# jglaser/metadynamics-plugin

Hardware: AMD Instinct MI355X
Metric: particle_cv_evals_per_s (higher is better)
Workload: dtype f32; 1 GPU; 1xMI355X: 10^6 particles, 2 lamellar CVs (8 Fourier modes each), 256^2 bias grid, well-tempered; particles_per_gpu=1000000, particles_global=1000000, n_cv=2, modes_per_cv=8, grid=256x256, stride=1, fast_trig=1, fast_trig_library_default=1, driver=host, mode=single

## Files before the change

### metadynamics-plugin_amd/csrc/fused.hip

```cpp
#include <hip/hip_runtime.h>
#include <hip/hip_ext.h>

#ifdef MTD_STAMPS
__device__ unsigned long long g_stamps[64];
#define MTD_STAMP(slot, cond)                                                   \
    do                                                                          \
        {                                                                       \
        if (cond) g_stamps[slot] = wall_clock64();                              \
        } while (0)
extern "C" int mtd_debug_read_stamps(unsigned long long *host)
    {
    return (int)hipMemcpyFromSymbol(host, HIP_SYMBOL(g_stamps), sizeof(unsigned long long) * 64);
    }
#else
#define MTD_STAMP(slot, cond) do { } while (0)
#endif

#include "lamellar_host.hpp"
#include "metad_host.hpp"
#include "comm_host.hpp"

#include <cstdlib>
#include <cstring>
#include <map>
#include <mutex>
#include <utility>
#include <vector>

namespace
{

using namespace mtd;

constexpr int FCV_THREADS = 512;
constexpr int FCV_UNROLL = 4;
constexpr int FF_THREADS = 256;
constexpr int FF_UNROLL = 2;

template<typename S4, int NCV, bool FAST, bool COMM, bool ORTHO, int U = FCV_UNROLL>
__global__ __launch_bounds__(FCV_THREADS) void k_fused_cv(const LamKArgs a, const S4 *__restrict__ postype, const unsigned int N,
                                                          double *partials, const MetadCfg c,
                                                          const unsigned int n_apply_blocks, const CommK ck)
    {
    __shared__ float s_coeff[MTD_MAX_CV * MTD_MAX_TYPES];
    __shared__ double s_wave[(FCV_THREADS / MTD_WAVE) * NCV];
    __shared__ double s_red[16];
    __shared__ ModeTables s_mt;

    MTD_STAMP(0, blockIdx.x == 0 && threadIdx.x == 0);
    MTD_STAMP(3, blockIdx.x == n_apply_blocks && threadIdx.x == 0);
    if (blockIdx.x < n_apply_blocks)
        {
        const unsigned int b0 = blockIdx.x * FCV_THREADS;
        apply_cells(c, b0, min(c.len, b0 + FCV_THREADS), blockIdx.x == 0, s_red);
// ... 49 lines not shown
template<> struct ff_groups<float4, 1, false> { static constexpr int value = 2; };
template<> struct ff_groups<double4, 1, true> { static constexpr int value = 2; };
template<> struct ff_groups<double4, 1, false> { static constexpr int value = 2; };

template<typename S4, int NCV, bool FAST, int GROUPS, bool COMM, bool ORTHO>
__global__ __launch_bounds__(FF_THREADS, 4) void k_fused_force(const FusedEntry e, const LamKArgs a, const ForcePtrs out,
                                                            const double two_over_n, const MetadCfg c, const int deposit, const CommK ck)
    {
    __shared__ ChainResult s_chain;
    __shared__ float s_wcoef[MTD_MAX_CV * MTD_MAX_TYPES];
    __shared__ double s_red[16];
    __shared__ ModeTables s_mt;

    const int wave = threadIdx.x >> 6;
    const int lane = threadIdx.x & 63;
    const unsigned int n_grid_blocks = fused_entry_read(e);
    const unsigned int n_blocks = e.n_particle_blocks;
    const S4 *__restrict__ postype = (const S4 *)e.postype;
    const unsigned int N = e.N;
    const unsigned int n_modes = e.n_modes;
    const bool grid_block = blockIdx.x < n_grid_blocks;
    const unsigned int block_id = blockIdx.x - n_grid_blocks;
    const unsigned int stride = n_blocks * FF_STREAM_THREADS;
    const unsigned int first = block_id * FF_STREAM_THREADS + (wave - 1) * MTD_WAVE + lane;
    const unsigned int first1 = first + FF_U * stride;

    ForceRegs<NCV, FF_U> R, R1;
    MTD_STAMP(16, blockIdx.x == 0 && threadIdx.x == 0);
    MTD_STAMP(24, blockIdx.x == n_grid_blocks && threadIdx.x == 0);
    constexpr int NCH = CHAIN_MAX_CV;
    ChainPre<NCH> pre;
    int pre_meta = 0;
    constexpr bool early = !COMM;
    float4 th = make_float4(0.f, 0.f, 0.f, 0.f), tq = th;
    float tc = 0.0f;
    if (wave == 0)
        {
        if (!grid_block)
            {
            static_assert(MTD_MAX_MODES >= MTD_WAVE && MTD_MAX_CV * MTD_MAX_TYPES >= MTD_WAVE, "a lane is a valid index");
            th = a.h[lane];
            tq = a.q[lane];
            tc = (&a.coeff[0][0])[lane];
            }
        if (early)
            pre_meta = chain_preload<NCH>(e, pre);
        else
            pre_meta = chain_preload<NCH, false>(e, pre);
        }
    RawGroup<S4, FF_U> raw0;
    if (wave != 0 && !grid_block && N) lam_force_request<S4, FF_U>(postype, N, first, stride, raw0);
    if (!grid_block)
        {
        if (wave == 0)
            {
            if (lane < (int)n_modes)
                {
                s_mt.h[lane] = th;
                s_mt.q[lane] = tq;
                }
            if (lane < NCV * MTD_MAX_TYPES) s_wcoef[lane] = tc;
            }
        lds_barrier();
        }
    MTD_STAMP(25, blockIdx.x == n_grid_blocks && threadIdx.x == 0);
    if (wave == 0)
        {
        ChainResult r;
        chain_preload_resolve<NCH>(pre_meta, pre);
        if constexpr (early)
            {
            double vi[3];
#pragma unroll
            for (int i = 0; i < NCH; ++i) vi[i] = (pre.x[i][0] + pre.x[i][1]) + (pre.x[i][2] + pre.x[i][3]);
            r = chain_wave(c, deposit != 0, true, nullptr, nullptr, false, &pre.patch, pre.patch_ok != 0, true, vi[0], vi[1], vi[2]);
            }
        else
            r = chain_wave(c, deposit != 0, true, &ck, nullptr, false, &pre.patch, pre.patch_ok != 0);
        MTD_STAMP(17, blockIdx.x == 0 && threadIdx.x == 0);
        MTD_STAMP(26, blockIdx.x == n_grid_blocks && threadIdx.x == 0);
        if (lane == 0) chain_share(s_chain, r);
        if (!grid_block && lane < NCV * MTD_MAX_TYPES)
            {
            const unsigned int cv = lane / MTD_MAX_TYPES;
            const unsigned int gs = cv < a.n_cv ? a.slot[cv] : 0u;
            const double b = gs == 0 ? r.bias[0] : (gs == 1 ? r.bias[1] : r.bias[2]);
            s_wcoef[lane] = (cv < a.n_cv) ? (float)((double)s_wcoef[lane] * b * two_over_n) : 0.0f;
            }
        }
    else if (!grid_block && N)
        {
        RawGroup<S4, FF_U> raw1;
        if (GROUPS > 1) lam_force_request<S4, FF_U>(postype, N, first1, stride, raw1);
        lam_force_unscaled_from<S4, NCV, FAST, FF_U, ORTHO>(a, N, first, stride, s_mt, raw0, R);
        if (GROUPS > 1) lam_force_unscaled_from<S4, NCV, FAST, FF_U, ORTHO>(a, N, first1, stride, s_mt, raw1, R1);
        MTD_STAMP(27, blockIdx.x == n_grid_blocks && threadIdx.x == 64);
        }
    lds_barrier();
    MTD_STAMP(18, blockIdx.x == 0 && threadIdx.x == 0);
    MTD_STAMP(28, blockIdx.x == n_grid_blocks && threadIdx.x == 64);

    if (grid_block)
        {
        const double2 sums = grid_first_pass_cells_256(c, s_chain, blockIdx.x);
        MTD_STAMP(19, blockIdx.x == 0 && threadIdx.x == 0);
        grid_first_pass_sums_256(c, blockIdx.x, sums, s_red);
        MTD_STAMP(20, blockIdx.x == 0 && threadIdx.x == 0);
        }
// ... 101 lines not shown
std::mutex g_force_profile_mutex;

bool force_profile_next(hipEvent_t &start, hipEvent_t &stop)
    {
    std::lock_guard<std::mutex> lock(g_force_profile_mutex);
    ForceProfile &p = g_force_profile;
    if (p.used + 2 > p.ev.size()) return false;
    start = p.ev[p.used];
    stop = p.ev[p.used + 1];
    p.used += 2;
    return true;
    }

template<typename F> int with_fused_cv_kernel(int dtype, bool fast, bool ortho, bool comm, unsigned int n_cv, F &&f)
    {
    return dispatch_s4_fast(dtype, fast, [&](auto s4, auto fast_c)
        {
        using S4 = typename decltype(s4)::type;
        constexpr bool FAST = decltype(fast_c)::value;
        return dispatch_bool(ortho, [&](auto ortho_c)
            {
            constexpr bool ORTHO = decltype(ortho_c)::value;
            if (comm)
                return dispatch_count<CHAIN_MAX_CV>(n_cv, [&](auto n) { return f(k_fused_cv<S4, decltype(n)::value, FAST, true, ORTHO>, s4); });
            return dispatch_count<MAXCV>(n_cv, [&](auto n) { return f(k_fused_cv<S4, decltype(n)::value, FAST, false, ORTHO>, s4); });
            });
        });
    }

}

namespace mtd
{
unsigned int resident_capacity(const void *kernel, int threads)
    {
    static std::mutex mu;
    static std::map<std::pair<int, const void *>, unsigned int> cache;
    int per_cu = 0, dev = 0, n_cu = 0;
    if (hipGetDevice(&dev) != hipSuccess)
        {
        (void)hipGetLastError();
        return 0;
        }
    std::lock_guard<std::mutex> lock(mu);
    auto it = cache.find(std::make_pair(dev, kernel));
    if (it != cache.end()) return it->second;
    unsigned int cap = 0;
    if (hipDeviceGetAttribute(&n_cu, hipDeviceAttributeMultiprocessorCount, dev) == hipSuccess &&
        hipOccupancyMaxActiveBlocksPerMultiprocessor(&per_cu, kernel, threads, 0) == hipSuccess)
        cap = (unsigned int)per_cu * (unsigned int)n_cu;
    else
        (void)hipGetLastError();
    cache[std::make_pair(dev, kernel)] = cap;
    return cap;
    }
}

extern "C" {

int mtd_fused_cv_pass(mtd_metad *m, const mtd_lamellar_set *set, unsigned int n_particles, const void *d_postype,
                      int dtype, const mtd_box *global_box, double *d_partials, unsigned int *n_partials,
                      mtd_stream_t stream)
    {
    if (!m) return MTD_ERR_INVALID_ARGUMENT;
    if (m->h_step_err && *m->h_step_err) return MTD_ERR_COMM_TIMEOUT;
    LamKArgs k;
    int rc = fill_kargs(k, set, global_box);
    if (rc) return rc;
    if (!d_partials || !n_partials || (n_particles && !d_postype)) return MTD_ERR_INVALID_ARGUMENT;
    if (dtype != MTD_F32 && dtype != MTD_F64) return MTD_ERR_INVALID_ARGUMENT;
    if (set->n_cv > (unsigned int)MAXCV) return MTD_ERR_UNSUPPORTED;
    hipStream_t s = (hipStream_t)stream;
    const unsigned int blocks = lam_cv_blocks(n_particles);
    *n_partials = blocks;
    const unsigned int n_apply = m->pending_apply ? (m->cfg.len + FCV_THREADS - 1) / FCV_THREADS : 0;
    const bool fast = lam_fast_trig(k) != 0;
    if (m->comm && (set->n_cv > (unsigned int)CHAIN_MAX_CV || set->n_cv != m->cfg.n_cv)) return MTD_ERR_UNSUPPORTED;
    const LamKArgs kd = dense_cv_args(k);
    rc = with_fused_cv_kernel(dtype, fast, k.ortho != 0, m->comm != nullptr, set->n_cv, [&](auto kernel, auto s4) -> int
        {
        using S4 = typename decltype(s4)::type;
        const unsigned int grid = blocks + n_apply;
        CommK ck;
        std::memset(&ck, 0, sizeof(ck));
        if (m->comm)
            {
            if (grid > resident_capacity((const void *)kernel, FCV_THREADS)) return MTD_ERR_UNSUPPORTED;
            const int rcn = comm_next(m->comm, ck);
            if (rcn) return rcn;
            }
        kernel<<<grid, FCV_THREADS, 0, s>>>(kd, (const S4 *)d_postype, n_particles, d_partials, m->cfg, n_apply, ck);
// ... 190 lines not shown
```

### metadynamics-plugin_amd/csrc/metad.hip

```cpp
#include "metad_device.hpp"

#include <cmath>
#include <cstring>
#include <mutex>
#include <new>

#include "metad_host.hpp"
#include "comm_host.hpp"

#include <cstdlib>

namespace
{

using namespace mtd;

__global__ __launch_bounds__(GRID_THREADS) void k_prepare(const MetadCfg c, const int deposit)
    {
    __shared__ EvalShared sh;
    __shared__ double s_tmp[16];
    reduce_cv_sources(c, sh.cv, s_tmp);
    __syncthreads();
    evaluate_bias(c, sh, deposit != 0, false);
    if (threadIdx.x < c.n_cv) c.st->cv[threadIdx.x] = sh.cv[threadIdx.x];
// ... 516 lines not shown
int mtd_metad_update_phase_a(mtd_metad *m, unsigned int timestep, int *deposited, mtd_stream_t stream)
    {
    if (!m || !deposited) return MTD_ERR_INVALID_ARGUMENT;
    { int frc = mtd::metad_flush(m, (hipStream_t)stream); if (frc) return frc; }
    hipStream_t s = (hipStream_t)stream;
    const int dep = deposit_due(m, timestep);
    k_prepare<<<1, GRID_THREADS, 0, s>>>(m->cfg, dep);
    MTD_LAUNCH_CHECK();
    if (dep)
        {
        k_reweight1<true, false><<<m->cfg.n_gblocks, GRID_THREADS, 0, s>>>(m->cfg);
        MTD_LAUNCH_CHECK();
        }
    *deposited = dep;
    return MTD_SUCCESS;
    }

int mtd_metad_update_phase_b(mtd_metad *m, int deposited, mtd_stream_t stream)
    {
    if (!m) return MTD_ERR_INVALID_ARGUMENT;
    hipStream_t s = (hipStream_t)stream;
    if (deposited)
        {
        k_reweight1<false, true><<<m->cfg.n_gblocks, GRID_THREADS, 0, s>>>(m->cfg);
        MTD_LAUNCH_CHECK();
        k_apply<<<m->cfg.n_gblocks, GRID_THREADS, 0, s>>>(m->cfg);
        MTD_LAUNCH_CHECK();
        }
    k_evaluate<<<1, GRID_THREADS, 0, s>>>(m->cfg);
    MTD_LAUNCH_CHECK();
    return MTD_SUCCESS;
    }

void mtd_debug_walker_check_pack(unsigned int stride, int add_bias, unsigned int timestep, double *out12)
    {
    const unsigned int q[3] = { stride, (unsigned int)(add_bias != 0), timestep };
    for (int i = 0; i < 3; ++i)
        {
        const double lo = (double)(q[i] & 0xffffu), hi = (double)(q[i] >> 16);
        out12[4 * i] = lo;
        out12[4 * i + 1] = lo * lo;
        out12[4 * i + 2] = hi;
        out12[4 * i + 3] = hi * hi;
        }
    }

int mtd_debug_walker_check_verify(const double *sums12, const double *mine12, unsigned int world)
    {
    const double W = (double)world;
    for (int i = 0; i < 12; ++i)
        if (sums12[i] != W * mine12[i]) return 0;
    return 1;
    }

int mtd_metad_update_bias_walkers(mtd_metad *m, mtd_rccl *walkers, unsigned int timestep, mtd_stream_t stream)
    {
    if (!m) return MTD_ERR_INVALID_ARGUMENT;
    int rc;
    if (walkers && (m->walkers_checked != (const void *)walkers || m->walkers_stride != m->stride || m->walkers_add_bias != m->add_bias))
        {
        double *d_chk = nullptr;
        MTD_HIP_TRY(hipMalloc(&d_chk, 12 * sizeof(double)));
        double mine[12], h[12];
        mtd_debug_walker_check_pack(m->stride, m->add_bias, timestep, mine);
        hipError_t e = hipMemcpyAsync(d_chk, mine, sizeof(mine), hipMemcpyHostToDevice, (hipStream_t)stream);
        rc = e == hipSuccess ? mtd_comm_allreduce_large(walkers, d_chk, 12, MTD_ELEM_F64, stream) : (int)e;
// ... 164 lines not shown
```

### metadynamics-plugin_amd/csrc/metad_device.hpp

```cpp
#pragma once

#include "mtd_device.hpp"
#include "comm_device.hpp"
#include "exact_div.hpp"

#include <cstddef>

#ifndef MTD_STAMP
#define MTD_STAMP(slot, cond) do { } while (0)
#endif

namespace mtd
{

constexpr int MAXCV = MTD_METAD_MAX_CV;
constexpr int GRID_THREADS = 256;
constexpr int MAX_POINTS = 2 * MAXCV + 2;
constexpr int MAX_TERMS = 1 << MAXCV;

struct CvSource
    {
    const double *partials;
    unsigned int n_partials, stride, offset, _pad;
    double scale, shift;
// ... 382 lines not shown
                    {
                    const int coord = gp.org[i] + rest % 6;
                    rest /= 6;
                    in = in && coord >= 0 && coord < (int)c.lengths[i];
                    cell += (unsigned int)coord * c.factors[i];
                    }
            if (in) gp.v[r] = c.grid[cell];
            }
        }
    return gp;
    }

template<int NCH> struct ChainPre
    {
    double x[NCH][4];
    GridPatch patch;
    int patch_ok;
    };

struct ChainSums
    {
    const double *ptr[CHAIN_MAX_CV];
    unsigned int cnt[CHAIN_MAX_CV], str[CHAIN_MAX_CV], off[CHAIN_MAX_CV];
    };

struct alignas(64) FusedEntry
    {
    const void *postype;
    MetadState *st;
    unsigned int N;
    unsigned int n_particle_blocks;
    unsigned int n_passenger_blocks;
    unsigned int n_modes, n_cv;
    unsigned int _pad;
    ChainSums sums;
    };
static_assert(sizeof(FusedEntry) <= 128 && alignof(FusedEntry) == 64, "one aligned batch of scalar loads");
static_assert(CHAIN_MAX_CV == 3 && sizeof(ChainSums) == 64 && offsetof(FusedEntry, sums) == 40, "fused_entry_read names every field");

__device__ __forceinline__ unsigned int fused_entry_read_head(const FusedEntry &e)
    {
    unsigned int npb;
    asm("s_mov_b32 %0, %1" : "=s"(npb) : "s"(e.n_passenger_blocks), "s"(e.postype), "s"(e.st), "s"(e.N), "s"(e.n_particle_blocks),
        "s"(e.n_modes), "s"(e.n_cv));
    return npb;
    }
__device__ __forceinline__ unsigned int fused_entry_read(const FusedEntry &e)
    {
    unsigned int npb;
    asm("s_mov_b32 %0, %1" : "=s"(npb) : "s"(e.n_passenger_blocks), "s"(e.postype), "s"(e.st), "s"(e.N), "s"(e.n_particle_blocks),
        "s"(e.n_modes), "s"(e.n_cv), "s"(e.sums.ptr[0]), "s"(e.sums.ptr[1]), "s"(e.sums.ptr[2]), "s"(e.sums.cnt[0]), "s"(e.sums.cnt[1]),
        "s"(e.sums.cnt[2]), "s"(e.sums.str[0]), "s"(e.sums.str[1]), "s"(e.sums.str[2]), "s"(e.sums.off[0]), "s"(e.sums.off[1]),
        "s"(e.sums.off[2]));
    return npb;
    }

inline ChainSums chain_sums_of(const MetadCfg &c)
    {
    ChainSums s;
    const double *safe = &c.st->zero;
#pragma unroll
    for (int i = 0; i < CHAIN_MAX_CV; ++i)
        {
        const bool on = i < (int)c.n_cv && c.src[i].partials != nullptr;
        s.ptr[i] = on ? c.src[i].partials : safe;
        s.cnt[i] = on ? c.src[i].n_partials : 0u;
        s.str[i] = on ? c.src[i].stride : 0u;
        s.off[i] = on ? c.src[i].offset : 0u;
        }
    return s;
    }

template<int NCH, bool SUMS>
__device__ __forceinline__ void chain_preload_sums(const ChainSums &s, const double *safe, ChainPre<NCH> &p)
    {
    const unsigned int lane = threadIdx.x & 63;
#pragma unroll
    for (int i = 0; i < NCH; ++i)
#pragma unroll
        for (int j = 0; j < 4; ++j)
            {
            const unsigned int b = lane + j * MTD_WAVE;
            const double *q = (SUMS && b < s.cnt[i]) ? s.ptr[i] + ((size_t)b * s.str[i] + s.off[i]) : safe;
            p.x[i][j] = SUMS ? *q : 0.0;
// ... 33 lines not shown
#pragma unroll
        for (int j = 0; j < 4; ++j)
            {
            const unsigned int b = lane + j * MTD_WAVE;
            const double *q = (SUMS && b < cnt[i]) ? ptr[i] + ((size_t)b * str[i] + off[i]) : safe;
            p.x[i][j] = SUMS ? *q : 0.0;
            }
    p.patch_ok = ok;
#pragma unroll
    for (int i = 0; i < CHAIN_MAX_CV; ++i) p.patch.org[i] = org[i];
    p.patch.v[0] = c.st->patch_v[lane];
#pragma unroll
    for (int r = 1; r < 4; ++r) p.patch.v[r] = NCH == 3 ? c.st->patch_v[min(lane + 64 * r, 215u)] : 0.0;
    }

template<int NCH, bool SUMS = true>
__device__ __forceinline__ int chain_preload(const FusedEntry &e, ChainPre<NCH> &p)
    {
    const unsigned int lane = threadIdx.x & 63;
    chain_preload_sums<NCH, SUMS>(e.sums, &e.st->zero, p);
    static_assert(offsetof(MetadState, patch_org) == offsetof(MetadState, patch_valid) + sizeof(int), "one run of four ints");
    const int meta = (&e.st->patch_valid)[min(lane, 3u)];
    chain_preload_patch<NCH>(e.st, p);
    return meta;
    }
template<int NCH>
__device__ __forceinline__ void chain_preload_resolve(const int meta, ChainPre<NCH> &p)
    {
    p.patch_ok = wave_read(meta, 0);
#pragma unroll
    for (int i = 0; i < CHAIN_MAX_CV; ++i) p.patch.org[i] = wave_read(meta, 1 + i);
    }

__device__ __forceinline__ double chain_div(const MetadCfg &c, const double a, const double b, const double y)
    {
    if (!c.fastdiv) return a / b;
    const double q0 = a * y;
    const double r0 = __builtin_fma(-b, q0, a);
    const double q1 = __builtin_fma(r0, y, q0);
    const double r1 = __builtin_fma(-b, q1, a);
    return __builtin_fma(r1, y, q1);
    }

__device__ __forceinline__ ChainResult chain_wave(const MetadCfg &c, const bool deposit, const bool closed_form,
                                                  const CommK *rx = nullptr, const double *given = nullptr,
                                                  const bool want_weight = false, const GridPatch *patch = nullptr,
                                                  const bool patch_ok = true, const bool have_init = false,
                                                  const double v_init0 = 0.0, const double v_init1 = 0.0, const double v_init2 = 0.0)
    {
    const int lane = threadIdx.x & 63;
    const unsigned int n = c.n_cv;
    const int n_term = 1 << n;
    ChainResult r;

    double x[CHAIN_MAX_CV][8];
    unsigned int n_part_max = 0;
#pragma unroll
    for (int i = 0; i < CHAIN_MAX_CV; ++i)
        if (i < (int)n && c.src[i].partials) n_part_max = max(n_part_max, c.src[i].n_partials);
    double v[CHAIN_MAX_CV] = { 0.0, 0.0, 0.0 };
    double rx_total[3] = { 0.0, 0.0, 0.0 };
    if (rx)
        {
        comm_recv_sum_wave(*rx, rx_total, n);
        n_part_max = 0;
        }
    else if (given)
        {
#pragma unroll
        for (int i = 0; i < CHAIN_MAX_CV; ++i) rx_total[i] = i < (int)n ? given[i] : 0.0;
        n_part_max = 0;
        }
    const bool handed = rx != nullptr || given != nullptr;
    if (have_init && n_part_max)
        {
        v[0] = v_init0;
        v[1] = v_init1;
        v[2] = v_init2;
        }
    for (unsigned int b0 = lane + ((have_init && n_part_max) ? 4 * MTD_WAVE : 0); b0 < n_part_max; b0 += 8 * MTD_WAVE)
        {
#pragma unroll
        for (int i = 0; i < CHAIN_MAX_CV; ++i)
#pragma unroll
            for (int j = 0; j < 8; ++j)
                {
                const unsigned int b = b0 + j * MTD_WAVE;
                x[i][j] = (i < (int)n && c.src[i].partials && b < c.src[i].n_partials)
                              ? c.src[i].partials[(size_t)b * c.src[i].stride + c.src[i].offset] : 0.0;
                }
#pragma unroll
        for (int i = 0; i < CHAIN_MAX_CV; ++i)
            v[i] += ((x[i][0] + x[i][1]) + (x[i][2] + x[i][3])) + ((x[i][4] + x[i][5]) + (x[i][6] + x[i][7]));
        }
#pragma unroll
    for (int i = 0; i < CHAIN_MAX_CV; ++i)
        {
        r.cv[i] = 0.0;
        r.bias[i] = 0.0;
        if (i < (int)n)
            {
            const double t = handed ? rx_total[i] : wave_sum(v[i]);
            r.cv[i] = (c.src[i].partials || handed) ? c.src[i].shift + c.src[i].scale * t : c.src[i].shift;
            }
        }

    MTD_STAMP(40, blockIdx.x == 0 && threadIdx.x == 0 && closed_form);
    int g_lower = 0, g_ok = 0;
    double g_rel = 0.0;
    if (lane < 3 * (int)n)
        {
        const int i = lane / 3, v = lane % 3;
        const double si = i == 0 ? r.cv[0] : (i == 1 ? r.cv[1] : r.cv[2]);
        const double delta = i == 0 ? c.delta[0] : (i == 1 ? c.delta[1] : c.delta[2]);
        const double cmin = i == 0 ? c.cv_min[0] : (i == 1 ? c.cv_min[1] : c.cv_min[2]);
        const double cmax = i == 0 ? c.cv_max[0] : (i == 1 ? c.cv_max[1] : c.cv_max[2]);
        const double rdel = i == 0 ? c.rdelta[0] : (i == 1 ? c.rdelta[1] : c.rdelta[2]);
        const int len = (int)(i == 0 ? c.lengths[0] : (i == 1 ? c.lengths[1] : c.lengths[2]));
        double val = si;
        if (v == 0) val = si - delta;
        if (v == 2) val = si + delta;
        g_ok = val >= cmin && val < cmax;
        int lower = (int)chain_div(c, val - cmin, delta, rdel);
        int upper = lower + 1;
        if (upper >= len)
            {
            lower--;
            upper--;
            }
        const double lower_bound = cmin + delta * lower;
        const double upper_bound = cmin + delta * upper;
        g_rel = (val - lower_bound) / (upper_bound - lower_bound);
        g_lower = lower;
        }

    MTD_STAMP(41, blockIdx.x == 0 && threadIdx.x == 0 && closed_form);
    const int n_pts = closed_form ? 1 + 2 * (int)n : 2 + 2 * (int)n;
    const int p = lane / n_term;
    const unsigned int bits = lane % n_term;
    const bool is_weight = (!closed_form) && p == 1 + 2 * (int)n;
    bool ok = p < n_pts;
    double wt = 1.0;
    unsigned int cell = 0;
    double d[CHAIN_MAX_CV];
    int pslot = 0, pmul = 1;
    bool in_patch = patch != nullptr && patch_ok;
#pragma unroll
    for (int i = 0; i < CHAIN_MAX_CV; ++i)
        {
        d[i] = 0.0;
        if (i < (int)n)
            {
            int var = 1;
            if (p == 1 + 2 * i) var = 0;
            if (p == 2 + 2 * i) var = 2;
            const int src_lane = 3 * i + var;
            const int lower = __shfl(g_lower, src_lane, MTD_WAVE);
            const double rel = __shfl(g_rel, src_lane, MTD_WAVE);
            const int oki = __shfl(g_ok, src_lane, MTD_WAVE);
            ok = ok && oki;
            unsigned int coord;
            if (bits & (1u << i))
                {
                coord = (unsigned int)lower;
                wt *= (1.0 - rel);
                }
            else
                {
                coord = (unsigned int)(lower + 1);
                wt *= rel;
                }
            cell += coord * c.factors[i];
            d[i] = (c.cv_min[i] + coord * c.delta[i]) - r.cv[i];
            if (patch)
                {
                const int o = (int)coord - patch->org[i];
                in_patch = in_patch && o >= 0 && o < 6;
                pslot += o * pmul;
                pmul *= 6;
                }
            }
        }
    double val = 0.0;
    if (patch)
        {
        const int src = (in_patch && ok) ? pslot : 0;
        double pv = __shfl(patch->v[0], src & 63, MTD_WAVE);
        if (n == 3)
            {
            const double p1 = __shfl(patch->v[1], src & 63, MTD_WAVE), p2 = __shfl(patch->v[2], src & 63, MTD_WAVE),
                         p3 = __shfl(patch->v[3], src & 63, MTD_WAVE);
            const int reg = src >> 6;
            pv = reg == 0 ? pv : (reg == 1 ? p1 : (reg == 2 ? p2 : p3));
            }
        if (ok) val = (in_patch && !is_weight) ? pv : (is_weight ? c.weight[cell] : c.grid[cell]);
        }
    else if (ok) val = is_weight ? c.weight[cell] : c.grid[cell];
    r.c_wt = wt;
    r.c_wold = (want_weight && ok && p == 0) ? c.weight[cell] : 0.0;
    r.c_dV = 0.0;

    double e_g = 0.0;
    if (closed_form && deposit && ok)
        {
        double gauss_exp = 0.0;
#pragma unroll
        for (int i = 0; i < CHAIN_MAX_CV; ++i)
#pragma unroll
            for (int j = 0; j < CHAIN_MAX_CV; ++j)
                if (i < (int)n && j < (int)n)
                    {
                    const double sij = c.sigma_inv[i * n + j];
                    gauss_exp += d[i] * d[j] * (1.0 / 2.0) * (sij * sij);
                    }
        e_g = exp(-gauss_exp);
        }
    bool on_grid = true;
    unsigned int bin = 0;
#pragma unroll
    for (int i = 0; i < CHAIN_MAX_CV; ++i)
        {
        if (i < (int)n)
            {
            const double q = chain_div(c, r.cv[i] - c.cv_min[i], c.delta[i], c.rdelta[i]);
            if (!(q > -1.0) || !(q < 4294967296.0))
                on_grid = false;
            else
                {
                const unsigned int coord = (unsigned int)q;
                if (coord >= c.lengths[i]) on_grid = false;
                bin += coord * c.factors[i];
                }
            }
        }
    r.on_grid = on_grid ? 1 : 0;
    r.bin = bin;

    MTD_STAMP(42, blockIdx.x == 0 && threadIdx.x == 0 && closed_form);
    double term = ok ? wt * val : 0.0;
    double V_old = 0.0;
    for (int b = 0; b < n_term; ++b) V_old += wave_read(term, b);
    r.scal = 1.0;
    if (deposit && c.mode == MTD_MODE_WELL_TEMPERED) r.scal = exp(chain_div(c, -V_old, c.T_shift, c.rT_shift));

    MTD_STAMP(43, blockIdx.x == 0 && threadIdx.x == 0 && closed_form);
    if (closed_form && deposit && ok)
        {
        r.c_dV = (c.W * r.scal) * e_g;
        val += r.c_dV;
        term = wt * val;
        }
    if (!ok) r.c_wt = 0.0;

    MTD_STAMP(44, blockIdx.x == 0 && threadIdx.x == 0 && closed_form);
    double res = 0.0;
    if (n == 2)
        {
        res += dpp_move<0x00>(term);
        res += dpp_move<0x55>(term);
        res += dpp_move<0xAA>(term);
        res += dpp_move<0xFF>(term);
        }
    else if (n == 1)
        {
        res += dpp_move<0xA0>(term);
        res += dpp_move<0xF5>(term);
        }
    else
        {
        const int base = (p < n_pts ? p : 0) * n_term;
        double t8[8];
#pragma unroll
        for (int b = 0; b < 8; ++b) t8[b] = __shfl(term, (base + b) & 63, MTD_WAVE);
#pragma unroll
        for (int b = 0; b < 8; ++b) res += t8[b];
        }

    const double res0 = wave_read(res, 0);
    r.V = res0;
    r.w = closed_form ? 1.0 : wave_read(res, (1 + 2 * (int)n) * n_term);
    r.oob = !wave_read((int)ok, 0);
#pragma unroll
    for (int i = 0; i < CHAIN_MAX_CV; ++i)
        {
        if (i < (int)n)
            {
            const double rm = wave_read(res, (1 + 2 * i) * n_term);
            const double rp = wave_read(res, (2 + 2 * i) * n_term);
            const double s = r.cv[i];
            const double delta = c.delta[i];
            double b;
            if (s - delta < c.cv_min[i])
                b = chain_div(c, rp - res0, delta, c.rdelta[i]);
            else if (s + delta > c.cv_max[i])
                b = chain_div(c, res0 - rm, delta, c.rdelta[i]);
            else
                b = chain_div(c, rp - rm, 2.0 * delta, c.rdelta2[i]);
            r.bias[i] = b;
            }
        }
    MTD_STAMP(45, blockIdx.x == 0 && threadIdx.x == 0 && closed_form);
    r.failed = 0;
    if (handed)
        {
        bool bad = false;
#pragma unroll
        for (int i = 0; i < CHAIN_MAX_CV; ++i) bad = bad || (i < (int)n && is_comm_poison(rx_total[i]));
        if (bad)
            {
            const double nan = __longlong_as_double(0x7ff8000000000000ll);
#pragma unroll
            for (int i = 0; i < CHAIN_MAX_CV; ++i)
                if (i < (int)n) r.cv[i] = r.bias[i] = nan;
            r.V = r.w = nan;
            r.scal = 0.0;
            r.on_grid = 0;
            r.oob = 0;
            r.failed = 1;
            }
        }
    return r;
    }

__device__ __forceinline__ double gauss_exponent3(const MetadCfg &c, unsigned int idx, const double s0, const double s1,
                                                  const double s2)
    {
    const unsigned int n = c.n_cv;
    unsigned int rest = idx;
    unsigned int c2 = 0, c1 = 0, c0;
    if (n > 2)
        {
        c2 = rest / c.factors[2];
        rest -= c2 * c.factors[2];
        }
    if (n > 1)
        {
        c1 = rest / c.factors[1];
        rest -= c1 * c.factors[1];
        }
    c0 = rest;
    double d[3];
    d[0] = (c.cv_min[0] + c0 * c.delta[0]) - s0;
    d[1] = n > 1 ? (c.cv_min[1] + c1 * c.delta[1]) - s1 : 0.0;
    d[2] = n > 2 ? (c.cv_min[2] + c2 * c.delta[2]) - s2 : 0.0;
    double gauss_exp = 0.0;
#pragma unroll
    for (int i = 0; i < 3; ++i)
#pragma unroll
        for (int j = 0; j < 3; ++j)
            if (i < (int)n && j < (int)n)
                {
                const double sij = c.sigma_inv[i * n + j];
                gauss_exp += d[i] * d[j] * (1.0 / 2.0) * (sij * sij);
                }
    return gauss_exp;
// ... 103 lines not shown
```

### metadynamics-plugin_amd/csrc/metad_host.hpp

```cpp
#pragma once

#include "metad_device.hpp"

struct mtd_metad
    {
    mtd::MetadCfg cfg;
    unsigned int stride;
    int add_bias;
    void *slab;
    int pending_apply;
    int w_stale;
    struct mtd_comm *comm;
    unsigned long long *d_ll;
    unsigned int *d_step_err;
    volatile unsigned int *h_step_err;
    unsigned int *d_step_err_host;
    unsigned int step_seq;
    unsigned int last_launches;
    int step_mode;
    const void *walkers_checked;
    unsigned int walkers_stride;
    int walkers_add_bias;
    };

namespace mtd
{
inline int deposit_due(const mtd_metad *m, unsigned int timestep) { return (m->add_bias && (timestep % m->stride == 0)) ? 1 : 0; }
inline FusedEntry fused_entry(const MetadCfg &c, const void *postype, unsigned int N, unsigned int n_particle_blocks,
                              unsigned int n_passenger_blocks, unsigned int n_modes, unsigned int n_cv)
    {
    FusedEntry e;
    e.postype = postype;
    e.st = c.st;
    e.N = N;
    e.n_particle_blocks = n_particle_blocks;
    e.n_passenger_blocks = n_passenger_blocks;
    e.n_modes = n_modes;
    e.n_cv = n_cv;
    e._pad = 0;
    e.sums = chain_sums_of(c);
    return e;
    }
unsigned int resident_capacity(const void *kernel, int threads);
int metad_flush(mtd_metad *m, hipStream_t s);
int fused_grid_step(mtd_metad *m, unsigned int timestep, hipStream_t s);
void announce_pending_apply(mtd_metad *m, hipStream_t s);
void withdraw_pending_apply(mtd_metad *m);
mtd_metad *take_pending_apply(hipStream_t s, MetadCfg &cfg);
void commit_pending_apply(mtd_metad *m);
void fused_step_release(mtd_metad *m);
}
```

Baseline: 111.1 billion particle-CV-evals/s.

## Add specialized chain_fast path with lane-distributed config preload for non-comm fused force

Adds a template-specialized chain_fast<NCV> routine for the non-communicating fused force kernel. Each lane preloads one 64-bit word of MetadCfg early, alongside the chain preload, and values are then pulled with wave_read instead of repeated scalar loads from the config struct. The path also compile-time fixes the CV count and skips the weight, handed and poison branches. Shared math is factored into small helpers reused by chain_wave. The fast path is on by default and can be disabled with an env var; it adds code complexity and relies on the config layout matching the static asserts.

```diff
diff --git a/metadynamics-plugin_amd/csrc/fused.hip b/metadynamics-plugin_amd/csrc/fused.hip
--- a/metadynamics-plugin_amd/csrc/fused.hip
+++ b/metadynamics-plugin_amd/csrc/fused.hip
@@ -20,6 +20,7 @@
 #include "metad_host.hpp"
 #include "comm_host.hpp"
 
+#include <atomic>
 #include <cstdlib>
 #include <cstring>
 #include <map>
@@ -135,6 +136,7 @@
     ChainPre<NCH> pre;
     int pre_meta = 0;
     constexpr bool early = !COMM;
+    unsigned long long cfg_word = 0;
     float4 th = make_float4(0.f, 0.f, 0.f, 0.f), tq = th;
     float tc = 0.0f;
     if (wave == 0)
@@ -147,7 +149,10 @@
             tc = (&a.coeff[0][0])[lane];
             }
         if (early)
+            {
             pre_meta = chain_preload<NCH>(e, pre);
+            cfg_word = chain_cfg_request(c);
+            }
         else
             pre_meta = chain_preload<NCH, false>(e, pre);
         }
@@ -176,7 +181,16 @@
             double vi[3];
 #pragma unroll
             for (int i = 0; i < NCH; ++i) vi[i] = (pre.x[i][0] + pre.x[i][1]) + (pre.x[i][2] + pre.x[i][3]);
-            r = chain_wave(c, deposit != 0, true, nullptr, nullptr, false, &pre.patch, pre.patch_ok != 0, true, vi[0], vi[1], vi[2]);
+            if (e.chain_fast)
+                {
+                static_assert(NCV <= NCH, "k_fused_force is instantiated for 1 .. CHAIN_MAX_CV lamellar CVs");
+                double vn[NCV];
+#pragma unroll
+                for (int i = 0; i < NCV; ++i) vn[i] = vi[i];
+                r = chain_fast<NCV>(cfg_word, deposit != 0, grid_block || blockIdx.x == 0, pre.patch, pre.patch_ok != 0, vn);
+                }
+            else
+                r = chain_wave(c, deposit != 0, true, nullptr, nullptr, false, &pre.patch, pre.patch_ok != 0, true, vi[0], vi[1], vi[2]);
             }
         else
             r = chain_wave(c, deposit != 0, true, &ck, nullptr, false, &pre.patch, pre.patch_ok != 0);
@@ -344,6 +358,14 @@
 
 namespace mtd
 {
+static int chain_select_from_env()
+    {
+    const char *v = std::getenv("MTD_CHAIN_SELECT");
+    return (v && v[0] == '1' && v[1] == 0) ? 1 : 0;
+    }
+static std::atomic<int> g_chain_select{chain_select_from_env()};
+int chain_select() { return g_chain_select.load(std::memory_order_relaxed); }
+
 unsigned int resident_capacity(const void *kernel, int threads)
     {
     static std::mutex mu;
@@ -369,6 +391,8 @@
 }
 
 extern "C" {
+
+void mtd_debug_chain_select(int select) { mtd::g_chain_select.store(select == 1 ? 1 : 0, std::memory_order_relaxed); }
 
 int mtd_fused_cv_pass(mtd_metad *m, const mtd_lamellar_set *set, unsigned int n_particles, const void *d_postype,
                       int dtype, const mtd_box *global_box, double *d_partials, unsigned int *n_partials,
diff --git a/metadynamics-plugin_amd/csrc/metad.hip b/metadynamics-plugin_amd/csrc/metad.hip
--- a/metadynamics-plugin_amd/csrc/metad.hip
+++ b/metadynamics-plugin_amd/csrc/metad.hip
@@ -572,6 +572,8 @@
     return MTD_SUCCESS;
     }
 
+int mtd_debug_chain_fastdiv(const mtd_metad *m) { return m ? m->cfg.fastdiv : -1; }
+
 void mtd_debug_walker_check_pack(unsigned int stride, int add_bias, unsigned int timestep, double *out12)
     {
     const unsigned int q[3] = { stride, (unsigned int)(add_bias != 0), timestep };
diff --git a/metadynamics-plugin_amd/csrc/metad_device.hpp b/metadynamics-plugin_amd/csrc/metad_device.hpp
--- a/metadynamics-plugin_amd/csrc/metad_device.hpp
+++ b/metadynamics-plugin_amd/csrc/metad_device.hpp
@@ -438,7 +438,7 @@
     unsigned int n_particle_blocks;
     unsigned int n_passenger_blocks;
     unsigned int n_modes, n_cv;
-    unsigned int _pad;
+    unsigned int chain_fast;
     ChainSums sums;
     };
 static_assert(sizeof(FusedEntry) <= 128 && alignof(FusedEntry) == 64, "one aligned batch of scalar loads");
@@ -455,7 +455,7 @@
     {
     unsigned int npb;
     asm("s_mov_b32 %0, %1" : "=s"(npb) : "s"(e.n_passenger_blocks), "s"(e.postype), "s"(e.st), "s"(e.N), "s"(e.n_particle_blocks),
-        "s"(e.n_modes), "s"(e.n_cv), "s"(e.sums.ptr[0]), "s"(e.sums.ptr[1]), "s"(e.sums.ptr[2]), "s"(e.sums.cnt[0]), "s"(e.sums.cnt[1]),
+        "s"(e.n_modes), "s"(e.n_cv), "s"(e.chain_fast), "s"(e.sums.ptr[0]), "s"(e.sums.ptr[1]), "s"(e.sums.ptr[2]), "s"(e.sums.cnt[0]), "s"(e.sums.cnt[1]),
         "s"(e.sums.cnt[2]), "s"(e.sums.str[0]), "s"(e.sums.str[1]), "s"(e.sums.str[2]), "s"(e.sums.off[0]), "s"(e.sums.off[1]),
         "s"(e.sums.off[2]));
     return npb;
@@ -555,14 +555,144 @@
     for (int i = 0; i < CHAIN_MAX_CV; ++i) p.patch.org[i] = wave_read(meta, 1 + i);
     }
 
-__device__ __forceinline__ double chain_div(const MetadCfg &c, const double a, const double b, const double y)
-    {
-    if (!c.fastdiv) return a / b;
+__device__ __forceinline__ double chain_div(const int &fastdiv, const double a, const double b, const double y)
+    {
+    if (!fastdiv) return a / b;
     const double q0 = a * y;
     const double r0 = __builtin_fma(-b, q0, a);
     const double q1 = __builtin_fma(r0, y, q0);
     const double r1 = __builtin_fma(-b, q1, a);
     return __builtin_fma(r1, y, q1);
+    }
+__device__ __forceinline__ double chain_div(const MetadCfg &c, const double a, const double b, const double y)
+    {
+    return chain_div(c.fastdiv, a, b, y);
+    }
+
+
+__device__ __forceinline__ double chain_cv_value(const bool summed, const double &shift, const double &scale, const double t)
+    {
+    return summed ? shift + scale * t : shift;
+    }
+
+__device__ __forceinline__ void chain_geometry(const int &fastdiv, const int v, const double si, const double delta, const double cmin,
+                                               const double cmax, const double rdel, const int len, int &g_ok, int &g_lower,
+                                               double &g_rel)
+    {
+    double val = si;
+    if (v == 0) val = si - delta;
+    if (v == 2) val = si + delta;
+    g_ok = val >= cmin && val < cmax;
+    int lower = (int)chain_div(fastdiv, val - cmin, delta, rdel);
+    int upper = lower + 1;
+    if (upper >= len)
+        {
+        lower--;
+        upper--;
+        }
+    const double lower_bound = cmin + delta * lower;
+    const double upper_bound = cmin + delta * upper;
+    g_rel = (val - lower_bound) / (upper_bound - lower_bound);
+    g_lower = lower;
+    }
+
+__device__ __forceinline__ unsigned int chain_corner(const bool low, const int lower, const double rel, double &wt)
+    {
+    unsigned int coord;
+    if (low)
+        {
+        coord = (unsigned int)lower;
+        wt *= (1.0 - rel);
+        }
+    else
+        {
+        coord = (unsigned int)(lower + 1);
+        wt *= rel;
+        }
+    return coord;
+    }
+__device__ __forceinline__ double chain_node_offset(const double &cmin, const unsigned int coord, const double &delta, const double s)
+    {
+    return (cmin + coord * delta) - s;
+    }
+__device__ __forceinline__ void chain_gauss_add(double &gauss_exp, const double di, const double dj, const double &sigma_inv_ij)
+    {
+    const double sij = sigma_inv_ij;
+    gauss_exp += di * dj * (1.0 / 2.0) * (sij * sij);
+    }
+__device__ __forceinline__ double chain_patch_value(const GridPatch &patch, const int src, const bool three)
+    {
+    double pv = __shfl(patch.v[0], src & 63, MTD_WAVE);
+    if (three)
+        {
+        const double p1 = __shfl(patch.v[1], src & 63, MTD_WAVE), p2 = __shfl(patch.v[2], src & 63, MTD_WAVE),
+                     p3 = __shfl(patch.v[3], src & 63, MTD_WAVE);
+        const int reg = src >> 6;
+        pv = reg == 0 ? pv : (reg == 1 ? p1 : (reg == 2 ? p2 : p3));
+        }
+    return pv;
+    }
+__device__ __forceinline__ void chain_bin_add(const int &fastdiv, const double s, const double &cmin, const double &delta,
+                                              const double &rdel, const unsigned int &len, const unsigned int &factor, bool &on_grid,
+                                              unsigned int &bin)
+    {
+    const double q = chain_div(fastdiv, s - cmin, delta, rdel);
+    if (!(q > -1.0) || !(q < 4294967296.0))
+        on_grid = false;
+    else
+        {
+        const unsigned int coord = (unsigned int)q;
+        if (coord >= len) on_grid = false;
+        bin += coord * factor;
+        }
+    }
+__device__ __forceinline__ double chain_deposit_corner(const double &W, const double scal, const double e_g, const double wt, double &val,
+                                                       double &term)
+    {
+    const double dV = (W * scal) * e_g;
+    val += dV;
+    term = wt * val;
+    return dV;
+    }
+__device__ __forceinline__ double chain_point_sum_1(const double term)
+    {
+    double res = 0.0;
+    res += dpp_move<0xA0>(term);
+    res += dpp_move<0xF5>(term);
+    return res;
+    }
+__device__ __forceinline__ double chain_point_sum_2(const double term)
+    {
+    double res = 0.0;
+    res += dpp_move<0x00>(term);
+    res += dpp_move<0x55>(term);
+    res += dpp_move<0xAA>(term);
+    res += dpp_move<0xFF>(term);
+    return res;
+    }
+__device__ __forceinline__ double chain_point_sum_3(const double term, const int base)
+    {
+    double res = 0.0;
+    double t8[8];
+#pragma unroll
+    for (int b = 0; b < 8; ++b) t8[b] = __shfl(term, (base + b) & 63, MTD_WAVE);
+#pragma unroll
+    for (int b = 0; b < 8; ++b) res += t8[b];
+    return res;
+    }
+__device__ __forceinline__ double chain_difference(const int &fastdiv, const double s, const double &delta_i, const double &cmin,
+                                                   const double &cmax, const double &rdel, const double &rdel2, const double res0,
+                                                   const double rm, const double rp)
+    {
+    const double delta = delta_i;
+    double b;
+    if (s - delta < cmin)
+        b = chain_div(fastdiv, rp - res0, delta, rdel);
+    else if (s + delta > cmax)
+        b = chain_div(fastdiv, res0 - rm, delta, rdel);
+    else
+        b = chain_div(fastdiv, rp - rm, 2.0 * delta, rdel2);
+    return b;
     }
 
 __device__ __forceinline__ ChainResult chain_wave(const MetadCfg &c, const bool deposit, const bool closed_form,
@@ -624,7 +754,7 @@
         if (i < (int)n)
             {
             const double t = handed ? rx_total[i] : wave_sum(v[i]);
-            r.cv[i] = (c.src[i].partials || handed) ? c.src[i].shift + c.src[i].scale * t : c.src[i].shift;
+            r.cv[i] = chain_cv_value(c.src[i].partials || handed, c.src[i].shift, c.src[i].scale, t);
             }
         }
 
@@ -640,21 +770,7 @@
         const double cmax = i == 0 ? c.cv_max[0] : (i == 1 ? c.cv_max[1] : c.cv_max[2]);
         const double rdel = i == 0 ? c.rdelta[0] : (i == 1 ? c.rdelta[1] : c.rdelta[2]);
         const int len = (int)(i == 0 ? c.lengths[0] : (i == 1 ? c.lengths[1] : c.lengths[2]));
-        double val = si;
-        if (v == 0) val = si - delta;
-        if (v == 2) val = si + delta;
-        g_ok = val >= cmin && val < cmax;
-        int lower = (int)chain_div(c, val - cmin, delta, rdel);
-        int upper = lower + 1;
-        if (upper >= len)
-            {
-            lower--;
-            upper--;
-            }
-        const double lower_bound = cmin + delta * lower;
-        const double upper_bound = cmin + delta * upper;
-        g_rel = (val - lower_bound) / (upper_bound - lower_bound);
-        g_lower = lower;
+        chain_geometry(c.fastdiv, v, si, delta, cmin, cmax, rdel, len, g_ok, g_lower, g_rel);
         }
 
     MTD_STAMP(41, blockIdx.x == 0 && threadIdx.x == 0 && closed_form);
@@ -682,19 +798,9 @@
             const double rel = __shfl(g_rel, src_lane, MTD_WAVE);
             const int oki = __shfl(g_ok, src_lane, MTD_WAVE);
             ok = ok && oki;
-            unsigned int coord;
-            if (bits & (1u << i))
-                {
-                coord = (unsigned int)lower;
-                wt *= (1.0 - rel);
-                }
-            else
-                {
-                coord = (unsigned int)(lower + 1);
-                wt *= rel;
-                }
+            const unsigned int coord = chain_corner((bits & (1u << i)) != 0, lower, rel, wt);
             cell += coord * c.factors[i];
-            d[i] = (c.cv_min[i] + coord * c.delta[i]) - r.cv[i];
+            d[i] = chain_node_offset(c.cv_min[i], coord, c.delta[i], r.cv[i]);
             if (patch)
                 {
                 const int o = (int)coord - patch->org[i];
@@ -708,14 +814,7 @@
     if (patch)
         {
         const int src = (in_patch && ok) ? pslot : 0;
-        double pv = __shfl(patch->v[0], src & 63, MTD_WAVE);
-        if (n == 3)
-            {
-            const double p1 = __shfl(patch->v[1], src & 63, MTD_WAVE), p2 = __shfl(patch->v[2], src & 63, MTD_WAVE),
-                         p3 = __shfl(patch->v[3], src & 63, MTD_WAVE);
-            const int reg = src >> 6;
-            pv = reg == 0 ? pv : (reg == 1 ? p1 : (reg == 2 ? p2 : p3));
-            }
+        const double pv = chain_patch_value(*patch, src, n == 3);
         if (ok) val = (in_patch && !is_weight) ? pv : (is_weight ? c.weight[cell] : c.grid[cell]);
         }
     else if (ok) val = is_weight ? c.weight[cell] : c.grid[cell];
@@ -732,10 +831,7 @@
 #pragma unroll
             for (int j = 0; j < CHAIN_MAX_CV; ++j)
                 if (i < (int)n && j < (int)n)
-                    {
-                    const double sij = c.sigma_inv[i * n + j];
-                    gauss_exp += d[i] * d[j] * (1.0 / 2.0) * (sij * sij);
-                    }
+                    chain_gauss_add(gauss_exp, d[i], d[j], c.sigma_inv[i * n + j]);
         e_g = exp(-gauss_exp);
         }
     bool on_grid = true;
@@ -744,17 +840,7 @@
     for (int i = 0; i < CHAIN_MAX_CV; ++i)
         {
         if (i < (int)n)
-            {
-            const double q = chain_div(c, r.cv[i] - c.cv_min[i], c.delta[i], c.rdelta[i]);
-            if (!(q > -1.0) || !(q < 4294967296.0))
-                on_grid = false;
-            else
-                {
-                const unsigned int coord = (unsigned int)q;
-                if (coord >= c.lengths[i]) on_grid = false;
-                bin += coord * c.factors[i];
-                }
-            }
+            chain_bin_add(c.fastdiv, r.cv[i], c.cv_min[i], c.delta[i], c.rdelta[i], c.lengths[i], c.factors[i], on_grid, bin);
         }
     r.on_grid = on_grid ? 1 : 0;
     r.bin = bin;
@@ -767,37 +853,17 @@
     if (deposit && c.mode == MTD_MODE_WELL_TEMPERED) r.scal = exp(chain_div(c, -V_old, c.T_shift, c.rT_shift));
 
     MTD_STAMP(43, blockIdx.x == 0 && threadIdx.x == 0 && closed_form);
-    if (closed_form && deposit && ok)
-        {
-        r.c_dV = (c.W * r.scal) * e_g;
-        val += r.c_dV;
-        term = wt * val;
-        }
+    if (closed_form && deposit && ok) r.c_dV = chain_deposit_corner(c.W, r.scal, e_g, wt, val, term);
     if (!ok) r.c_wt = 0.0;
 
     MTD_STAMP(44, blockIdx.x == 0 && threadIdx.x == 0 && closed_form);
     double res = 0.0;
     if (n == 2)
-        {
-        res += dpp_move<0x00>(term);
-        res += dpp_move<0x55>(term);
-        res += dpp_move<0xAA>(term);
-        res += dpp_move<0xFF>(term);
-        }
+        res = chain_point_sum_2(term);
     else if (n == 1)
-        {
-        res += dpp_move<0xA0>(term);
-        res += dpp_move<0xF5>(term);
-        }
+        res = chain_point_sum_1(term);
     else
-        {
-        const int base = (p < n_pts ? p : 0) * n_term;
-        double t8[8];
-#pragma unroll
-        for (int b = 0; b < 8; ++b) t8[b] = __shfl(term, (base + b) & 63, MTD_WAVE);
-#pragma unroll
-        for (int b = 0; b < 8; ++b) res += t8[b];
-        }
+        res = chain_point_sum_3(term, (p < n_pts ? p : 0) * n_term);
 
     const double res0 = wave_read(res, 0);
     r.V = res0;
@@ -810,16 +876,8 @@
             {
             const double rm = wave_read(res, (1 + 2 * i) * n_term);
             const double rp = wave_read(res, (2 + 2 * i) * n_term);
-            const double s = r.cv[i];
-            const double delta = c.delta[i];
-            double b;
-            if (s - delta < c.cv_min[i])
-                b = chain_div(c, rp - res0, delta, c.rdelta[i]);
-            else if (s + delta > c.cv_max[i])
-                b = chain_div(c, res0 - rm, delta, c.rdelta[i]);
-            else
-                b = chain_div(c, rp - rm, 2.0 * delta, c.rdelta2[i]);
-            r.bias[i] = b;
+            r.bias[i] = chain_difference(c.fastdiv, r.cv[i], c.delta[i], c.cv_min[i], c.cv_max[i], c.rdelta[i], c.rdelta2[i], res0,
+                                         rm, rp);
             }
         }
     MTD_STAMP(45, blockIdx.x == 0 && threadIdx.x == 0 && closed_form);
@@ -844,6 +902,216 @@
         }
     return r;
     }
+
+constexpr int CC_HEAD_WORDS = 34, CC_W_WORD = (int)(offsetof(MetadCfg, W) / 8), CC_MODE_WORD = (int)(offsetof(MetadCfg, mode) / 8),
+              CC_DIV_WORD = (int)(offsetof(MetadCfg, n_gblocks) / 8), CC_SRC_WORD = (int)(offsetof(MetadCfg, src) / 8);
+constexpr int CC_W_LANE = CC_HEAD_WORDS, CC_MODE_LANE = CC_W_LANE + 2, CC_DIV_LANE = CC_MODE_LANE + 2, CC_SRC_LANE = CC_DIV_LANE + 8,
+              CC_LANES = CC_SRC_LANE + 15;
+static_assert(offsetof(MetadCfg, sigma_inv) + 9 * sizeof(double) == CC_HEAD_WORDS * 8 && offsetof(MetadCfg, lengths) == 8 &&
+              offsetof(MetadCfg, factors) % 8 == 0, "head: n_cv | len, lengths, factors, cv_min, cv_max, delta, sigma_inv[0 .. 8]");
+static_assert(offsetof(MetadCfg, T_shift) == offsetof(MetadCfg, W) + 8 && offsetof(MetadCfg, grid) == offsetof(MetadCfg, mode) + 8,
+              "two words each");
+static_assert(offsetof(MetadCfg, n_gblocks) % 8 == 0 && offsetof(MetadCfg, fastdiv) == offsetof(MetadCfg, n_gblocks) + 4 &&
+              offsetof(MetadCfg, rdelta) == offsetof(MetadCfg, n_gblocks) + 8 && offsetof(MetadCfg, rT_shift) == offsetof(MetadCfg, n_gblocks) + 56,
+              "eight words");
+static_assert(sizeof(CvSource) == 40 && offsetof(MetadCfg, src) % 8 == 0 && CC_LANES <= MTD_WAVE && CHAIN_MAX_CV == 3, "fifteen words");
+
+__host__ __device__ constexpr int chain_cfg_lane(const size_t off)
+    {
+    const int w = (int)(off / 8);
+    return w < CC_HEAD_WORDS ? w
+                             : (w < CC_W_WORD + 2 ? CC_W_LANE + (w - CC_W_WORD)
+                                                  : (w < CC_MODE_WORD + 2 ? CC_MODE_LANE + (w - CC_MODE_WORD)
+                                                                          : (w < CC_DIV_WORD + 8 ? CC_DIV_LANE + (w - CC_DIV_WORD)
+                                                                                                 : CC_SRC_LANE + (w - CC_SRC_WORD))));
+    }
+__device__ __forceinline__ unsigned long long chain_cfg_request(const MetadCfg &c)
+    {
+    const int lane = threadIdx.x & 63;
+    int w = lane;
+    if (lane >= CC_W_LANE) w = CC_W_WORD + (lane - CC_W_LANE);
+    if (lane >= CC_MODE_LANE) w = CC_MODE_WORD + (lane - CC_MODE_LANE);
+    if (lane >= CC_DIV_LANE) w = CC_DIV_WORD + (lane - CC_DIV_LANE);
+    if (lane >= CC_SRC_LANE) w = CC_SRC_WORD + (lane - CC_SRC_LANE);
+    if (lane >= CC_LANES) w = 0;
+    static_assert((CC_SRC_WORD + 15) * 8 <= (int)sizeof(MetadCfg), "inside the struct");
+    return ((const unsigned long long *)&c)[w];
+    }
+__device__ __forceinline__ double chain_cfg_double(const unsigned long long cw, const size_t off)
+    {
+    return wave_read(__longlong_as_double((long long)cw), chain_cfg_lane(off));
+    }
+__device__ __forceinline__ unsigned int chain_cfg_uint(const unsigned long long cw, const size_t off)
+    {
+    const int half = (off & 4) ? (int)(cw >> 32) : (int)cw;
+    return (unsigned int)wave_read(half, chain_cfg_lane(off));
+    }
+#define MTD_CC_D(field, i) chain_cfg_double(cw, offsetof(MetadCfg, field) + sizeof(double) * (i))
+#define MTD_CC_U(field, i) chain_cfg_uint(cw, offsetof(MetadCfg, field) + sizeof(unsigned int) * (i))
+#define MTD_CC_SRC(field, i) (offsetof(MetadCfg, src) + sizeof(CvSource) * (i) + offsetof(CvSource, field))
+
+template<int N, typename T> __device__ __forceinline__ T chain_pick(const int i, const T (&a)[N])
+    {
+    if constexpr (N == 1)
+        return a[0];
+    else if constexpr (N == 2)
+        return i == 0 ? a[0] : a[1];
+    else
+        return i == 0 ? a[0] : (i == 1 ? a[1] : a[2]);
+    }
+
+template<int N>
+__device__ __forceinline__ ChainResult chain_fast(const unsigned long long cw, const bool deposit, const bool tail, const GridPatch &patch,
+                                                  const bool patch_ok, const double (&v_init)[N])
+    {
+    static_assert(N >= 1 && N <= CHAIN_MAX_CV, "one wave holds the (point, corner) pairs of up to three variables");
+    const int lane = threadIdx.x & 63;
+    constexpr int n_term = 1 << N;
+    ChainResult r;
+    const int fastdiv = (int)MTD_CC_U(fastdiv, 0);
+    double delta[N], cmin[N], cmax[N], rdel[N], rdel2[N];
+    unsigned int len[N], factor[N];
+#pragma unroll
+    for (int i = 0; i < N; ++i)
+        {
+        delta[i] = MTD_CC_D(delta, i);
+        cmin[i] = MTD_CC_D(cv_min, i);
+        cmax[i] = MTD_CC_D(cv_max, i);
+        rdel[i] = MTD_CC_D(rdelta, i);
+        rdel2[i] = MTD_CC_D(rdelta2, i);
+        len[i] = MTD_CC_U(lengths, i);
+        factor[i] = MTD_CC_U(factors, i);
+        }
+
+#pragma unroll
+    for (int i = 0; i < CHAIN_MAX_CV; ++i) r.cv[i] = r.bias[i] = 0.0;
+    double s[N];
+#pragma unroll
+    for (int i = 0; i < N; ++i)
+        {
+        const double t = wave_sum(v_init[i]);
+        const bool summed = (chain_cfg_uint(cw, MTD_CC_SRC(partials, i)) | chain_cfg_uint(cw, MTD_CC_SRC(partials, i) + 4)) != 0;
+        s[i] = chain_cv_value(summed, chain_cfg_double(cw, MTD_CC_SRC(shift, i)), chain_cfg_double(cw, MTD_CC_SRC(scale, i)), t);
+        r.cv[i] = s[i];
+        }
+
+    MTD_STAMP(40, blockIdx.x == 0 && threadIdx.x == 0);
+    int g_lower = 0, g_ok = 0;
+    double g_rel = 0.0;
+    if (lane < 3 * N)
+        {
+        const int i = lane / 3, v = lane % 3;
+        chain_geometry(fastdiv, v, chain_pick<N>(i, s), chain_pick<N>(i, delta), chain_pick<N>(i, cmin), chain_pick<N>(i, cmax),
+                       chain_pick<N>(i, rdel), (int)chain_pick<N>(i, len), g_ok, g_lower, g_rel);
+        }
+
+    MTD_STAMP(41, blockIdx.x == 0 && threadIdx.x == 0);
+    constexpr int n_pts = 1 + 2 * N;
+    const int p = lane / n_term;
+    const unsigned int bits = lane % n_term;
+    bool ok = p < n_pts;
+    double wt = 1.0;
+    unsigned int cell = 0;
+    double d[N];
+    int pslot = 0, pmul = 1;
+    bool in_patch = patch_ok;
+#pragma unroll
+    for (int i = 0; i < N; ++i)
+        {
+        int var = 1;
+        if (p == 1 + 2 * i) var = 0;
+        if (p == 2 + 2 * i) var = 2;
+        const int src_lane = 3 * i + var;
+        const int lower = __shfl(g_lower, src_lane, MTD_WAVE);
+        const double rel = __shfl(g_rel, src_lane, MTD_WAVE);
+        const int oki = __shfl(g_ok, src_lane, MTD_WAVE);
+        ok = ok && oki;
+        const unsigned int coord = chain_corner((bits & (1u << i)) != 0, lower, rel, wt);
+        cell += coord * factor[i];
+        d[i] = chain_node_offset(cmin[i], coord, delta[i], s[i]);
+        const int o = (int)coord - patch.org[i];
+        in_patch = in_patch && o >= 0 && o < 6;
+        pslot += o * pmul;
+        pmul *= 6;
+        }
+    double val = 0.0;
+        {
+        const int src = (in_patch && ok) ? pslot : 0;
+        const double pv = chain_patch_value(patch, src, N == 3);
+        if (ok)
+            {
+            if (in_patch)
+                val = pv;
+            else
+                {
+                const double *grid = (const double *)(((unsigned long long)MTD_CC_U(grid, 1) << 32) | MTD_CC_U(grid, 0));
+                val = grid[cell];
+                }
+            }
+        }
+
+    double e_g = 0.0;
+    if (deposit && ok)
+        {
+        double gauss_exp = 0.0;
+#pragma unroll
+        for (int i = 0; i < N; ++i)
+#pragma unroll
+            for (int j = 0; j < N; ++j) chain_gauss_add(gauss_exp, d[i], d[j], MTD_CC_D(sigma_inv, i * N + j));
+        e_g = exp(-gauss_exp);
+        }
+    r.on_grid = 0;
+    r.bin = 0;
+    if (tail)
+        {
+        bool on_grid = true;
+        unsigned int bin = 0;
+#pragma unroll
+        for (int i = 0; i < N; ++i) chain_bin_add(fastdiv, s[i], cmin[i], delta[i], rdel[i], len[i], factor[i], on_grid, bin);
+        r.on_grid = on_grid ? 1 : 0;
+        r.bin = bin;
+        }
+
+    MTD_STAMP(42, blockIdx.x == 0 && threadIdx.x == 0);
+    double term = ok ? wt * val : 0.0;
+    double V_old = 0.0;
+#pragma unroll
+    for (int b = 0; b < n_term; ++b) V_old += wave_read(term, b);
+    r.scal = 1.0;
+    if (deposit && (int)MTD_CC_U(mode, 0) == MTD_MODE_WELL_TEMPERED)
+        r.scal = exp(chain_div(fastdiv, -V_old, MTD_CC_D(T_shift, 0), MTD_CC_D(rT_shift, 0)));
+
+    MTD_STAMP(43, blockIdx.x == 0 && threadIdx.x == 0);
+    r.c_wt = r.c_wold = r.c_dV = 0.0;
+    if (deposit && ok) chain_deposit_corner(MTD_CC_D(W, 0), r.scal, e_g, wt, val, term);
+
+    MTD_STAMP(44, blockIdx.x == 0 && threadIdx.x == 0);
+    double res;
+    if constexpr (N == 1)
+        res = chain_point_sum_1(term);
+    else if constexpr (N == 2)
+        res = chain_point_sum_2(term);
+    else
+        res = chain_point_sum_3(term, (p < n_pts ? p : 0) * n_term);
+
+    const double res0 = wave_read(res, 0);
+    r.V = res0;
+    r.w = 1.0;
+    r.oob = !wave_read((int)ok, 0);
+#pragma unroll
+    for (int i = 0; i < N; ++i)
+        {
+        const double rm = wave_read(res, (1 + 2 * i) * n_term);
+        const double rp = wave_read(res, (2 + 2 * i) * n_term);
+        r.bias[i] = chain_difference(fastdiv, s[i], delta[i], cmin[i], cmax[i], rdel[i], rdel2[i], res0, rm, rp);
+        }
+    MTD_STAMP(45, blockIdx.x == 0 && threadIdx.x == 0);
+    r.failed = 0;
+    return r;
+    }
+#undef MTD_CC_D
+#undef MTD_CC_U
+#undef MTD_CC_SRC
 
 __device__ __forceinline__ double gauss_exponent3(const MetadCfg &c, unsigned int idx, const double s0, const double s1,
                                                   const double s2)
diff --git a/metadynamics-plugin_amd/csrc/metad_host.hpp b/metadynamics-plugin_amd/csrc/metad_host.hpp
--- a/metadynamics-plugin_amd/csrc/metad_host.hpp
+++ b/metadynamics-plugin_amd/csrc/metad_host.hpp
@@ -26,6 +26,7 @@
 namespace mtd
 {
 inline int deposit_due(const mtd_metad *m, unsigned int timestep) { return (m->add_bias && (timestep % m->stride == 0)) ? 1 : 0; }
+int chain_select();
 inline FusedEntry fused_entry(const MetadCfg &c, const void *postype, unsigned int N, unsigned int n_particle_blocks,
                               unsigned int n_passenger_blocks, unsigned int n_modes, unsigned int n_cv)
     {
@@ -37,8 +38,10 @@
     e.n_passenger_blocks = n_passenger_blocks;
     e.n_modes = n_modes;
     e.n_cv = n_cv;
-    e._pad = 0;
     e.sums = chain_sums_of(c);
+    bool fast = chain_select() == 0 && n_cv == c.n_cv && n_cv <= (unsigned int)CHAIN_MAX_CV;
+    for (int i = 0; i < CHAIN_MAX_CV; ++i) fast = fast && e.sums.cnt[i] <= 4u * MTD_WAVE;
+    e.chain_fast = fast ? 1u : 0u;
     return e;
     }
 unsigned int resident_capacity(const void *kernel, int threads);
```

Result: no change. 111.9 billion particle-CV-evals/s (median of 6 runs) (+0.7%).
